# mratsim/constantine

Measured on NVIDIA H100. Metric: bls12_381_g1_msm_throughput, higher is better.
Workload: dtype u32

## Files before the change

constantine_b200/csrc/msm_affine.cuh:

```cuda
#pragma once
#include "ec.cuh"
#include "field_inv.cuh"

namespace b200 {

constexpr int AFF_MAX_LEVELS = 8;
constexpr uint32_t AFF_NONE = 0xFFFFFFFFu;

static __global__ void k_bucket_bounds(const uint32_t* __restrict__ keys, size_t n, uint32_t no_key, uint32_t* head, uint32_t* tail) {
  size_t q = (size_t)blockIdx.x * blockDim.x + threadIdx.x;
  if (q >= n) return;
  const uint32_t key = keys[q];
  if (key >= no_key) return;
  if (q == 0 || keys[q - 1] != key) head[key] = (uint32_t)q;
  if (q + 1 == n || keys[q + 1] != key) tail[key] = (uint32_t)(q + 1);
}

constexpr int SCAN_THREADS = 256, SCAN_PER_THREAD = 4, SCAN_ITEMS = SCAN_THREADS * SCAN_PER_THREAD;

B200_DEV uint32_t block_exclusive_scan(uint32_t v, uint32_t& total, uint32_t* smem ) {
  const unsigned lane = threadIdx.x & 31u, warp = threadIdx.x >> 5;
  uint32_t inc = v;
#pragma unroll
  for (int d = 1; d < 32; d <<= 1) {
    uint32_t t = __shfl_up_sync(0xFFFFFFFFu, inc, d);
    if (lane >= (unsigned)d) inc += t;
  }
  __syncthreads();
  if (lane == 31u) smem[warp] = inc;
  __syncthreads();
  uint32_t base = 0, tot = 0;
#pragma unroll
  for (int w = 0; w < SCAN_THREADS / 32; w++) {
    const uint32_t s = smem[w];
    if ((unsigned)w < warp) base += s;
    tot += s;
  }
  total = tot;
  return base + inc - v;
}

B200_DEV uint32_t level_count(uint32_t n, int r) { return (n + (1u << r) - 1u) >> r; }

static __global__ void __launch_bounds__(SCAN_THREADS) k_level_blocksums(const uint32_t* __restrict__ head, const uint32_t* __restrict__ tail,
                                                                          uint32_t nb, int L, uint32_t nblk, uint32_t* blocksum ) {
  __shared__ uint32_t sm[SCAN_THREADS / 32 + 1];
  const uint32_t b0 = blockIdx.x * SCAN_ITEMS + threadIdx.x * SCAN_PER_THREAD;
  uint32_t cnt[SCAN_PER_THREAD];
#pragma unroll
  for (int k = 0; k < SCAN_PER_THREAD; k++) cnt[k] = (b0 + k < nb) ? tail[b0 + k] - head[b0 + k] : 0u;
  for (int r = 0; r <= L; r++) {
    uint32_t s = 0;
#pragma unroll
    for (int k = 0; k < SCAN_PER_THREAD; k++) s += level_count(cnt[k], r);
    uint32_t tot;
    block_exclusive_scan(s, tot, sm);
    if (threadIdx.x == 0) blocksum[(size_t)r * nblk + blockIdx.x] = tot;
  }
}

static __global__ void __launch_bounds__(SCAN_THREADS) k_level_scan(uint32_t* blocksum, uint32_t nblk, int L, uint32_t nb, uint32_t* off) {
  __shared__ uint32_t sm[SCAN_THREADS / 32 + 1];
  for (int r = 0; r <= L; r++) {
    uint32_t carry = 0;
    for (uint32_t base = 0; base < nblk; base += SCAN_THREADS) {
      const uint32_t i = base + threadIdx.x;
      const uint32_t v = (i < nblk) ? blocksum[(size_t)r * nblk + i] : 0u;
      uint32_t tot;
      const uint32_t ex = block_exclusive_scan(v, tot, sm);
      if (i < nblk) blocksum[(size_t)r * nblk + i] = carry + ex;
      carry += tot;
    }
    if (threadIdx.x == 0) off[(size_t)r * (nb + 1) + nb] = carry;
  }
}

static __global__ void __launch_bounds__(SCAN_THREADS) k_level_offsets(const uint32_t* __restrict__ head, const uint32_t* __restrict__ tail,
                                                                        uint32_t nb, int L, uint32_t nblk, const uint32_t* __restrict__ blocksum,
                                                                        uint32_t* off) {
  __shared__ uint32_t sm[SCAN_THREADS / 32 + 1];
  const uint32_t b0 = blockIdx.x * SCAN_ITEMS + threadIdx.x * SCAN_PER_THREAD;
  uint32_t cnt[SCAN_PER_THREAD];
#pragma unroll
  for (int k = 0; k < SCAN_PER_THREAD; k++) cnt[k] = (b0 + k < nb) ? tail[b0 + k] - head[b0 + k] : 0u;
  for (int r = 0; r <= L; r++) {
    uint32_t c[SCAN_PER_THREAD], s = 0;
#pragma unroll
    for (int k = 0; k < SCAN_PER_THREAD; k++) { c[k] = level_count(cnt[k], r); s += c[k]; }
    uint32_t tot;
    uint32_t ex = block_exclusive_scan(s, tot, sm) + blocksum[(size_t)r * nblk + blockIdx.x];
#pragma unroll
    for (int k = 0; k < SCAN_PER_THREAD; k++) {
      if (b0 + k < nb) off[(size_t)r * (nb + 1) + b0 + k] = ex;
      ex += c[k];
    }
  }
}

struct AffinePlan {
  uint2* plan0;
  uint32_t* plan[AFF_MAX_LEVELS];
  uint32_t* surv_keys;
  uint32_t* surv_vals;
};

static __global__ void k_affine_plan(const uint32_t* __restrict__ keys, const uint32_t* __restrict__ vals, size_t n, uint32_t no_key,
                                     const uint32_t* __restrict__ head, const uint32_t* __restrict__ tail,
                                     const uint32_t* __restrict__ off, uint32_t nb, int L, AffinePlan P) {
  size_t q = (size_t)blockIdx.x * blockDim.x + threadIdx.x;
  if (q >= n) return;
  const uint32_t b = keys[q];
  if (b >= no_key) return;
  const uint32_t h = head[b], i = (uint32_t)q - h, cnt = tail[b] - h;
  const size_t stride = (size_t)nb + 1;
  for (int r = 0; r < L; r++) {
    if (i & ((2u << r) - 1u)) break;
    const uint32_t p = off[(size_t)(r + 1) * stride + b] + (i >> (r + 1));
    const uint32_t s = i >> r;
    const bool has2 = s + 1u < level_count(cnt, r);
    if (r == 0) P.plan0[p] = make_uint2(vals[q], has2 ? vals[q + 1] : AFF_NONE);
    else P.plan[r][p] = (off[(size_t)r * stride + b] + s) | (has2 ? 0x80000000u : 0u);
  }
  if ((i & ((1u << L) - 1u)) == 0u) {
    const uint32_t ps = off[(size_t)L * stride + b] + (i >> L);
    P.surv_keys[ps] = b;
    P.surv_vals[ps] = ps;
  }
}

template <class T>
B200_DEV Aff<T> load_affine_rw(const uint32_t* base, size_t idx) {
  const uint32_t* p = base + idx * (2 * T::WORDS);
  Aff<T> a;
  load_words_rw(a.x, p);
  load_words_rw(a.y, p + T::WORDS);
  return a;
}
template <class T>
B200_DEV void store_affine(uint32_t* base, size_t idx, const Aff<T>& a) {
  uint32_t* p = base + idx * (2 * T::WORDS);
  store_words(p, a.x);
  store_words(p + T::WORDS, a.y);
}

template <class T>
B200_DEV void scratch_store(uint4* scratch, size_t threads, size_t tid, uint32_t j, const T& v) {
  constexpr int V = T::WORDS / 4;
#pragma unroll
  for (int k = 0; k < V; k++) {
    uint4 w;
    w.x = v.word(4 * k + 0); w.y = v.word(4 * k + 1); w.z = v.word(4 * k + 2); w.w = v.word(4 * k + 3);
    scratch[((size_t)j * V + k) * threads + tid] = w;
  }
}
template <class T>
B200_DEV T scratch_load(const uint4* scratch, size_t threads, size_t tid, uint32_t j) {
  constexpr int V = T::WORDS / 4;
  T v;
#pragma unroll
  for (int k = 0; k < V; k++) {
    const uint4 w = scratch[((size_t)j * V + k) * threads + tid];
    v.set_word(4 * k + 0, w.x); v.set_word(4 * k + 1, w.y); v.set_word(4 * k + 2, w.z); v.set_word(4 * k + 3, w.w);
  }
  return v;
}

constexpr int PART_TILE = 1024, PART_THREADS = 256, PART_MAX = 8;

B200_DEV uint32_t pair_chunk(const uint2 task, uint32_t n_points, uint32_t P) {
  uint32_t idx = task.x & 0x7FFFFFFFu;
  if (task.y != AFF_NONE) { const uint32_t j = task.y & 0x7FFFFFFFu; if (j > idx) idx = j; }
  uint32_t q = (uint32_t)(((unsigned long long)idx * P) / n_points);
  return q < P ? q : P - 1u;
}

static __global__ void __launch_bounds__(PART_THREADS) k_part_count(const uint2* __restrict__ plan0, const uint32_t* __restrict__ total_ptr,
                                                                    uint32_t n_points, uint32_t P, uint32_t nblk, uint32_t* counts) {
  __shared__ uint32_t sm[PART_MAX];
  if (threadIdx.x < PART_MAX) sm[threadIdx.x] = 0;
  __syncthreads();
  const uint32_t total = *total_ptr;
  const uint32_t base = blockIdx.x * PART_TILE;
  uint32_t local[PART_MAX];
#pragma unroll
  for (int q = 0; q < PART_MAX; q++) local[q] = 0;
  for (uint32_t i = threadIdx.x; i < PART_TILE; i += PART_THREADS) {
    const uint32_t p = base + i;
    if (p < total) {
      const uint32_t q = pair_chunk(plan0[p], n_points, P);
#pragma unroll
      for (int k = 0; k < PART_MAX; k++) local[k] += (q == (uint32_t)k) ? 1u : 0u;
    }
  }
#pragma unroll
  for (int q = 0; q < PART_MAX; q++) {
    uint32_t v = local[q];
    for (int d = 16; d >= 1; d >>= 1) v += __shfl_xor_sync(0xFFFFFFFFu, v, d);
    if ((threadIdx.x & 31u) == 0 && v) atomicAdd(&sm[q], v);
  }
  __syncthreads();
  if (threadIdx.x < P) counts[threadIdx.x * nblk + blockIdx.x] = sm[threadIdx.x];
}

static __global__ void __launch_bounds__(SCAN_THREADS) k_part_scan(uint32_t* counts, uint32_t P, uint32_t nblk, uint32_t* starts) {
  __shared__ uint32_t sm[SCAN_THREADS / 32 + 1];
  uint32_t carry = 0;
  const uint32_t len = P * nblk;
  for (uint32_t base = 0; base < len; base += SCAN_THREADS) {
    const uint32_t i = base + threadIdx.x;
    const uint32_t v = (i < len) ? counts[i] : 0u;
    uint32_t tot;
    const uint32_t ex = block_exclusive_scan(v, tot, sm);
    if (i < len) {
      counts[i] = carry + ex;
      if (i % nblk == 0) starts[i / nblk] = carry + ex;
    }
    carry += tot;
  }
  if (threadIdx.x == 0) starts[P] = carry;
}

static __global__ void __launch_bounds__(PART_THREADS) k_part_scatter(const uint2* __restrict__ plan0, const uint32_t* __restrict__ total_ptr,
                                                                      uint32_t n_points, uint32_t P, uint32_t nblk,
                                                                      const uint32_t* __restrict__ offsets, uint32_t* perm) {
  __shared__ uint32_t warp_cnt[PART_THREADS / 32][PART_MAX];
  __shared__ uint32_t run_base[PART_MAX];
  const uint32_t total = *total_ptr;
  const unsigned lane = threadIdx.x & 31u, warp = threadIdx.x >> 5;
  if (threadIdx.x < PART_MAX) run_base[threadIdx.x] = (threadIdx.x < P) ? offsets[threadIdx.x * nblk + blockIdx.x] : 0u;
  __syncthreads();
  for (uint32_t round = 0; round < PART_TILE / PART_THREADS; round++) {
    const uint32_t p = blockIdx.x * PART_TILE + round * PART_THREADS + threadIdx.x;
    const bool live = p < total;
    const uint32_t q = live ? pair_chunk(plan0[p], n_points, P) : 0xFFFFFFFFu;
    uint32_t my_rank = 0;
    for (uint32_t k = 0; k < P; k++) {
      const unsigned m = __ballot_sync(0xFFFFFFFFu, q == k);
      if (q == k) my_rank = __popc(m & ((1u << lane) - 1u));
      if (lane == 0) warp_cnt[warp][k] = __popc(m);
    }
    __syncthreads();
    if (live) {
      uint32_t before = 0;
      for (unsigned w = 0; w < warp; w++) before += warp_cnt[w][q];
      perm[run_base[q] + before + my_rank] = p;
    }
    __syncthreads();
    if (threadIdx.x < P) {
      uint32_t tot = 0;
      for (unsigned w = 0; w < PART_THREADS / 32; w++) tot += warp_cnt[w][threadIdx.x];
      run_base[threadIdx.x] += tot;
    }
    __syncthreads();
  }
}

enum PairKind { PAIR_COPY1 = 0, PAIR_COPY2 = 1, PAIR_INF = 2, PAIR_ADD = 3, PAIR_DBL = 4 };

struct PairTask {
  uint32_t a, b;
};
template <bool FIRST>
B200_DEV PairTask load_task(const void* plan, size_t p) {
  PairTask t;
  if constexpr (FIRST) {
    const uint2 v = reinterpret_cast<const uint2*>(plan)[p];
    t.a = v.x; t.b = v.y;
  } else {
    const uint32_t v = reinterpret_cast<const uint32_t*>(plan)[p];
    t.a = v & 0x7FFFFFFFu;
    t.b = (v >> 31) ? t.a + 1u : AFF_NONE;
  }
  return t;
}
template <class T, bool FIRST>
B200_DEV T load_x(const uint32_t* src, uint32_t ref) {
  T x;
  if constexpr (FIRST) load_words(x, src + (size_t)(ref & 0x7FFFFFFFu) * (2 * T::WORDS));
  else load_words_rw(x, src + (size_t)ref * (2 * T::WORDS));
  return x;
}
template <class T, bool FIRST>
B200_DEV void decode_y(T& y, uint32_t ref, bool& zero) {
  zero = y.is_zero();
  if constexpr (FIRST) y.cneg((ref >> 31) != 0);
}
template <class T, bool FIRST>
B200_DEV T load_y(const uint32_t* src, uint32_t ref, bool& zero) {
  T y;
  if constexpr (FIRST) load_words(y, src + (size_t)(ref & 0x7FFFFFFFu) * (2 * T::WORDS) + T::WORDS);
  else load_words_rw(y, src + (size_t)ref * (2 * T::WORDS) + T::WORDS);
  decode_y<T, FIRST>(y, ref, zero);
  return y;
}

template <class T>
B200_DEV int classify_pair(bool single, const T& x1, const T& y1, bool inf1, const T& x2, const T& y2, bool inf2, T& den) {
  if (single) return PAIR_COPY1;
  if (inf1) return PAIR_COPY2;
  if (inf2) return PAIR_COPY1;
  den = x2 - x1;
  if (!den.is_zero()) return PAIR_ADD;
  if (!(y1 == y2) || y1.is_zero()) return PAIR_INF;
  den = y1.dbl();
  return PAIR_DBL;
}

template <class T, bool FIRST>
B200_DEV void pair_factor(const uint32_t* src, uint32_t a, uint32_t b, const T& x1, const T& x2, T& run) {
  const bool single = b == AFF_NONE;
  T den = x2 - x1;
  bool contributes = !single;
  if (!single && (den.is_zero() || x1.is_zero() || x2.is_zero())) {
    bool z1, z2;
    const T y1 = load_y<T, FIRST>(src, a, z1), y2 = load_y<T, FIRST>(src, b, z2);
    const int kind = classify_pair(false, x1, y1, z1 && x1.is_zero(), x2, y2, z2 && x2.is_zero(), den);
    contributes = kind >= PAIR_ADD;
  }
  if (contributes) run = run.mul_u(den);
}

template <class T, class Prefix>
B200_DEV Aff<T> pair_result(const Aff<T>& P1, bool z1, const Aff<T>& P2, bool z2, bool single, uint32_t j, T& inv, Prefix prefix) {
  T den;
  const int kind = classify_pair(single, P1.x, P1.y, z1 && P1.x.is_zero(), P2.x, P2.y, z2 && P2.x.is_zero(), den);
  Aff<T> R;
  if (kind < PAIR_ADD) {
    if (kind == PAIR_COPY1) R = P1;
    else if (kind == PAIR_COPY2) R = P2;
    else { R.x = T::zero(); R.y = T::zero(); }
  } else {
    T inv_den = inv;
    if (j > 0) inv_den = inv.mul_u(prefix());
    inv = inv.mul_u(den);
    T num;
    if (kind == PAIR_ADD) num = P2.y - P1.y;
    else { const T xx = P1.x.sqr(); num = xx.dbl() + xx; }
    const T lam = num.mul_u(inv_den);
    R.x = lam.sqr_u() - P1.x - P2.x;
    R.y = lam.mul_u(P1.x - R.x) - P1.y;
  }
  return R;
}

#ifndef B200_AFF_THREADS
#define B200_AFF_THREADS 128
#endif
#ifndef B200_AFF_MIN_BLOCKS
#define B200_AFF_MIN_BLOCKS 4
#endif

B200_DEV void prefetch_l2(const void* p) { asm volatile("prefetch.global.L2 [%0];" ::"l"(p)); }
B200_DEV void prefetch_span(const void* p, int bytes) {
  prefetch_l2(p);
  prefetch_l2((const char*)p + bytes - 1);
}
template <class T, bool FIRST>
B200_DEV void prefetch_point(const uint32_t* src, uint32_t ref) {
  const uint32_t idx = FIRST ? (ref & 0x7FFFFFFFu) : ref;
  prefetch_span(src + (size_t)idx * (2 * T::WORDS), 2 * T::WORDS * 4);
}

__host__ __device__ __forceinline__ size_t pair_rows(size_t slots, size_t threads) { return (slots + threads - 1) / threads; }

struct PairSlots {
  const uint32_t* perm;
  uint32_t total, M;
  B200_DEV PairSlots(const uint32_t* total_ptr, const uint32_t* perm_, const uint32_t* range, size_t threads) {
    const uint32_t range_begin = range ? range[0] : 0u;
    total = range ? range[1] - range[0] : *total_ptr;
    perm = perm_;
    if (perm) perm += range_begin;
    M = (uint32_t)pair_rows(total, threads);
  }
  B200_DEV size_t first(size_t tid) const { return (tid & ~(size_t)31) * M + (tid & 31u); }
  B200_DEV uint32_t count(size_t tid) const {
    const size_t f = first(tid);
    if (f >= total) return 0u;
    const uint32_t c = (uint32_t)(((size_t)total - f + 31) / 32);
    return c < M ? c : M;
  }
  B200_DEV size_t slot(size_t tid, uint32_t j) const {
    const size_t t = first(tid) + 32u * (size_t)j;
    return perm ? (size_t)perm[t] : t;
  }
};

template <class T, bool FIRST>
__global__ void __launch_bounds__(B200_AFF_THREADS, (T::WORDS <= 12) ? B200_AFF_MIN_BLOCKS : 1)
k_affine_pairs(const void* __restrict__ plan, const uint32_t* __restrict__ total_ptr, const uint32_t* src, uint32_t* dst, uint4* scratch,
               const uint32_t* __restrict__ perm = nullptr, const uint32_t* __restrict__ range = nullptr) {
  const size_t threads = (size_t)gridDim.x * blockDim.x;
  const size_t tid = (size_t)blockIdx.x * blockDim.x + threadIdx.x;
  const PairSlots S(total_ptr, perm, range, threads);
  const unsigned lane = threadIdx.x & 31u;
  if (S.count(tid - lane) == 0) return;
  const uint32_t cnt = S.count(tid);
  T run = T::one();
  {
    PairTask t_next = cnt ? load_task<FIRST>(plan, S.slot(tid, 0)) : PairTask{0u, AFF_NONE};
    T x1n = T::zero(), x2n = T::zero();
    if (cnt) {
      x1n = load_x<T, FIRST>(src, t_next.a);
      if (t_next.b != AFF_NONE) x2n = load_x<T, FIRST>(src, t_next.b);
    }
#pragma unroll 1
    for (uint32_t j = 0; j < cnt; j++) {
      const PairTask t = t_next;
      const T x1 = x1n, x2 = x2n;
      if (j + 1 < cnt) {
        t_next = load_task<FIRST>(plan, S.slot(tid, j + 1));
        x1n = load_x<T, FIRST>(src, t_next.a);
        if (t_next.b != AFF_NONE) x2n = load_x<T, FIRST>(src, t_next.b);
      }
      pair_factor<T, FIRST>(src, t.a, t.b, x1, x2, run);
      scratch_store(scratch, threads, tid, j, run);
    }
  }
  T inv = fe_inverse(run);
  size_t p_prev = cnt ? S.slot(tid, cnt - 1) : 0;
  PairTask t_prev = cnt ? load_task<FIRST>(plan, p_prev) : PairTask{0u, AFF_NONE};
#pragma unroll 1
  for (uint32_t jj = cnt; jj > 0; jj--) {
    const uint32_t j = jj - 1;
    const size_t p = p_prev;
    const PairTask t = t_prev;
    if (j > 0) {
      p_prev = S.slot(tid, j - 1);
      t_prev = load_task<FIRST>(plan, p_prev);
      prefetch_point<T, FIRST>(src, t_prev.a);
      if (t_prev.b != AFF_NONE) prefetch_point<T, FIRST>(src, t_prev.b);
      if (j > 1) {
        constexpr int V = T::WORDS / 4;
#pragma unroll
        for (int k = 0; k < V; k++) prefetch_l2(scratch + ((size_t)(j - 2) * V + k) * threads + tid);
      }
    }
    const bool single = t.b == AFF_NONE;
    Aff<T> P1, P2;
    bool z1 = false, z2 = false;
    P1.x = load_x<T, FIRST>(src, t.a);
    P1.y = load_y<T, FIRST>(src, t.a, z1);
    if (!single) {
      P2.x = load_x<T, FIRST>(src, t.b);
      P2.y = load_y<T, FIRST>(src, t.b, z2);
    } else {
      P2.x = T::zero(); P2.y = T::zero();
    }
    store_affine(dst, p, pair_result(P1, z1, P2, z2, single, j, inv, [&] { return scratch_load<T>(scratch, threads, tid, j - 1); }));
  }
}

#ifndef B200_AFF_WS_CONSUMERS
#define B200_AFF_WS_CONSUMERS 8
#endif
#ifndef B200_AFF_WS_STAGES
#define B200_AFF_WS_STAGES 2
#endif
constexpr int AFF_WS_CONSUMERS = B200_AFF_WS_CONSUMERS;
constexpr int AFF_WS_THREADS = 32 * (AFF_WS_CONSUMERS + 1);

template <class T>
struct AffRing {
  static constexpr bool USED = T::WORDS <= 12;
  static constexpr int V = T::WORDS / 4;
  static constexpr int S2 = B200_AFF_WS_STAGES;
  static constexpr int ROWS = S2 * 5 * V;
  static constexpr int S1 = ROWS / (2 * V);
  static constexpr size_t BYTES = (size_t)AFF_WS_CONSUMERS * ROWS * 32 * 16;
};

B200_DEV uint32_t smem_addr(const void* p) { return (uint32_t)__cvta_generic_to_shared(p); }
B200_DEV void mbar_init(uint64_t* b, uint32_t count) { asm volatile("mbarrier.init.shared::cta.b64 [%0], %1;" ::"r"(smem_addr(b)), "r"(count) : "memory"); }
B200_DEV void mbar_arrive(uint64_t* b) { asm volatile("mbarrier.arrive.shared::cta.b64 _, [%0];" ::"r"(smem_addr(b)) : "memory"); }
B200_DEV void mbar_wait(uint64_t* b, uint32_t parity) {
  asm volatile(
      "{\n\t.reg .pred P1;\n"
      "WAIT:\n\t"
      "mbarrier.try_wait.parity.shared::cta.b64 P1, [%0], %1;\n\t"
      "@!P1 bra WAIT;\n\t}" ::"r"(smem_addr(b)),
      "r"(parity)
      : "memory");
}
B200_DEV void cp_async_arrive(uint64_t* b) { asm volatile("cp.async.mbarrier.arrive.noinc.shared::cta.b64 [%0];" ::"r"(smem_addr(b)) : "memory"); }
B200_DEV void cp_async16(void* s, const void* g) { asm volatile("cp.async.cg.shared.global [%0], [%1], 16;" ::"r"(smem_addr(s)), "l"(g) : "memory"); }

template <class T>
B200_DEV void ring_fetch(uint4* ring, int row, unsigned lane, const uint32_t* g) {
#pragma unroll
  for (int k = 0; k < T::WORDS / 4; k++) cp_async16(ring + (row + k) * 32 + lane, g + 4 * k);
}
template <class T>
B200_DEV T ring_load(const uint4* ring, int row, unsigned lane) {
  T v;
#pragma unroll
  for (int k = 0; k < T::WORDS / 4; k++) {
    const uint4 w = ring[(row + k) * 32 + lane];
    v.set_word(4 * k + 0, w.x); v.set_word(4 * k + 1, w.y); v.set_word(4 * k + 2, w.z); v.set_word(4 * k + 3, w.w);
  }
  return v;
}

template <class T, bool FIRST>
__global__ void __launch_bounds__(AFF_WS_THREADS, 1)
k_affine_pairs_ws(const void* __restrict__ plan, const uint32_t* __restrict__ total_ptr, const uint32_t* src, uint32_t* dst, uint4* scratch,
                  const uint32_t* __restrict__ perm = nullptr, const uint32_t* __restrict__ range = nullptr) {
  using RG = AffRing<T>;
  constexpr int V = RG::V, NC = AFF_WS_CONSUMERS, S1 = RG::S1, S2 = RG::S2;
  extern __shared__ __align__(16) unsigned char aff_ring_raw[];
  __shared__ uint64_t full1[NC][S1], empty1[NC][S1], full2[NC][S2], empty2[NC][S2], drained[NC];
  __shared__ uint32_t s_task[NC][S1][3][32];
  const unsigned lane = threadIdx.x & 31u, warp = threadIdx.x >> 5;
  if (threadIdx.x == 0) {
    for (int w = 0; w < NC; w++) {
      for (int s = 0; s < S1; s++) { mbar_init(&full1[w][s], 64); mbar_init(&empty1[w][s], 32); }
      for (int s = 0; s < S2; s++) { mbar_init(&full2[w][s], 64); mbar_init(&empty2[w][s], 32); }
      mbar_init(&drained[w], 32);
    }
  }
  __syncthreads();
  const size_t threads = (size_t)gridDim.x * NC * 32;
  const PairSlots S(total_ptr, perm, range, threads);
  uint4* const ring_base = reinterpret_cast<uint4*>(aff_ring_raw);

  if (warp == NC) {
    uint32_t n[NC], cnt[NC];
#pragma unroll
    for (int w = 0; w < NC; w++) {
      const size_t tid = ((size_t)blockIdx.x * NC + w) * 32 + lane;
      n[w] = S.count(tid - lane);
      cnt[w] = S.count(tid);
    }
    auto tid_of = [&](int w) { return ((size_t)blockIdx.x * NC + w) * 32 + lane; };
    auto src_of = [&](uint32_t ref) { return src + (size_t)(FIRST ? (ref & 0x7FFFFFFFu) : ref) * (2 * T::WORDS); };
    uint32_t ta[NC], tb[NC], tp[NC];
    auto fetch_task = [&](int w, uint32_t j) {
      const size_t p = S.slot(tid_of(w), j);
      const PairTask t = load_task<FIRST>(plan, p);
      ta[w] = t.a; tb[w] = t.b; tp[w] = (uint32_t)p;
    };
#pragma unroll
    for (int w = 0; w < NC; w++) if (cnt[w]) fetch_task(w, 0);
#pragma unroll 1
    for (uint32_t j = 0; j < n[0]; j++) {
      uint32_t ca[NC], cb[NC];
#pragma unroll
      for (int w = 0; w < NC; w++) { ca[w] = ta[w]; cb[w] = tb[w]; }
#pragma unroll
      for (int w = 0; w < NC; w++) if (j + 1 < cnt[w]) fetch_task(w, j + 1);
#pragma unroll
      for (int w = 0; w < NC; w++) {
        if (j >= n[w]) continue;
        const int s = (int)(j % S1);
        mbar_wait(&empty1[w][s], ((j / S1) & 1u) ^ 1u);
        uint4* ring = ring_base + (size_t)w * RG::ROWS * 32;
        if (j < cnt[w]) {
          s_task[w][s][0][lane] = ca[w];
          s_task[w][s][1][lane] = cb[w];
          ring_fetch<T>(ring, s * 2 * V, lane, src_of(ca[w]));
          if (cb[w] != AFF_NONE) ring_fetch<T>(ring, s * 2 * V + V, lane, src_of(cb[w]));
        }
        cp_async_arrive(&full1[w][s]);
        mbar_arrive(&full1[w][s]);
      }
    }
#pragma unroll
    for (int w = 0; w < NC; w++) if (n[w] && n[w] - 1 < cnt[w]) fetch_task(w, n[w] - 1);
#pragma unroll 1
    for (uint32_t jj = 0; jj < n[0]; jj++) {
      uint32_t ca[NC], cb[NC], cp[NC];
#pragma unroll
      for (int w = 0; w < NC; w++) { ca[w] = ta[w]; cb[w] = tb[w]; cp[w] = tp[w]; }
#pragma unroll
      for (int w = 0; w < NC; w++) if (jj + 1 < n[w] && n[w] - 2 - jj < cnt[w]) fetch_task(w, n[w] - 2 - jj);
#pragma unroll
      for (int w = 0; w < NC; w++) {
        if (jj >= n[w]) continue;
        if (jj == 0) mbar_wait(&drained[w], 0);
        const uint32_t j = n[w] - 1 - jj;
        const int s = (int)(jj % S2);
        mbar_wait(&empty2[w][s], ((jj / S2) & 1u) ^ 1u);
        uint4* ring = ring_base + (size_t)w * RG::ROWS * 32;
        if (j < cnt[w]) {
          s_task[w][s][0][lane] = ca[w];
          s_task[w][s][1][lane] = cb[w];
          s_task[w][s][2][lane] = cp[w];
          const int row = s * 5 * V;
          ring_fetch<T>(ring, row, lane, src_of(ca[w]));
          ring_fetch<T>(ring, row + V, lane, src_of(ca[w]) + T::WORDS);
          if (cb[w] != AFF_NONE) {
            ring_fetch<T>(ring, row + 2 * V, lane, src_of(cb[w]));
            ring_fetch<T>(ring, row + 3 * V, lane, src_of(cb[w]) + T::WORDS);
          }
          if (j > 0) {
#pragma unroll
            for (int k = 0; k < V; k++)
              cp_async16(ring + (row + 4 * V + k) * 32 + lane, scratch + ((size_t)(j - 1) * V + k) * threads + tid_of(w));
          }
        }
        cp_async_arrive(&full2[w][s]);
        mbar_arrive(&full2[w][s]);
      }
    }
    asm volatile("cp.async.wait_all;" ::: "memory");
    return;
  }

  const size_t tid = ((size_t)blockIdx.x * NC + warp) * 32 + lane;
  const uint32_t n = S.count(tid - lane), cnt = S.count(tid);
  if (n == 0) return;
  const uint4* ring = ring_base + (size_t)warp * RG::ROWS * 32;
  T run = T::one();
#pragma unroll 1
  for (uint32_t j = 0; j < n; j++) {
    const int s = (int)(j % S1);
    mbar_wait(&full1[warp][s], (j / S1) & 1u);
    const uint32_t a = s_task[warp][s][0][lane], b = s_task[warp][s][1][lane];
    const T x1 = ring_load<T>(ring, s * 2 * V, lane), x2 = ring_load<T>(ring, s * 2 * V + V, lane);
    mbar_arrive(&empty1[warp][s]);
    if (j >= cnt) continue;
    pair_factor<T, FIRST>(src, a, b, x1, x2, run);
    scratch_store(scratch, threads, tid, j, run);
  }
  mbar_arrive(&drained[warp]);
  T inv = fe_inverse(run);
#pragma unroll 1
  for (uint32_t jj = 0; jj < n; jj++) {
    const uint32_t j = n - 1 - jj;
    const int s = (int)(jj % S2);
    mbar_wait(&full2[warp][s], (jj / S2) & 1u);
    const int row = s * 5 * V;
    const uint32_t a = s_task[warp][s][0][lane], b = s_task[warp][s][1][lane], p = s_task[warp][s][2][lane];
    const bool single = b == AFF_NONE;
    Aff<T> P1, P2;
    P1.x = ring_load<T>(ring, row, lane);
    P1.y = ring_load<T>(ring, row + V, lane);
    P2.x = single ? T::zero() : ring_load<T>(ring, row + 2 * V, lane);
    P2.y = single ? T::zero() : ring_load<T>(ring, row + 3 * V, lane);
    const T pre = ring_load<T>(ring, row + 4 * V, lane);
    mbar_arrive(&empty2[warp][s]);
    if (j >= cnt) continue;
    bool z1, z2 = false;
    decode_y<T, FIRST>(P1.y, a, z1);
    if (!single) decode_y<T, FIRST>(P2.y, b, z2);
    store_affine(dst, p, pair_result(P1, z1, P2, z2, single, j, inv, [&] { return pre; }));
  }
}

template <class T>
struct PairKernel {
  static constexpr bool WS = AffRing<T>::USED;
  static constexpr int THREADS = WS ? AFF_WS_THREADS : B200_AFF_THREADS;
  static constexpr int SLOT_THREADS = WS ? 32 * AFF_WS_CONSUMERS : B200_AFF_THREADS;
  static constexpr int SMEM = WS ? (int)AffRing<T>::BYTES : 0;
  template <bool FIRST>
  static auto entry() {
    if constexpr (WS) return k_affine_pairs_ws<T, FIRST>;
    else return k_affine_pairs<T, FIRST>;
  }
};

template <class T>
cudaError_t affine_pairs_blocks_per_sm(int* bps) {
  using K = PairKernel<T>;
  int b[2] = {0, 0};
  cudaError_t e;
  for (int f = 0; f < 2; f++) {
    const auto k = f == 0 ? K::template entry<true>() : K::template entry<false>();
    if (K::SMEM && (e = cudaFuncSetAttribute(k, cudaFuncAttributeMaxDynamicSharedMemorySize, K::SMEM)) != cudaSuccess) return e;
    if ((e = cudaOccupancyMaxActiveBlocksPerMultiprocessor(&b[f], k, K::THREADS, K::SMEM)) != cudaSuccess) return e;
  }
  *bps = b[1] < b[0] ? b[1] : b[0];
  return cudaSuccess;
}

template <class T, bool FIRST>
void launch_affine_pairs(unsigned grid, cudaStream_t s, const void* plan, const uint32_t* total_ptr, const uint32_t* src, uint32_t* dst, uint4* scratch,
                         const uint32_t* perm = nullptr, const uint32_t* range = nullptr) {
  using K = PairKernel<T>;
  K::template entry<FIRST>()<<<grid, K::THREADS, K::SMEM, s>>>(plan, total_ptr, src, dst, scratch, perm, range);
}

}
```

Before: 114.7.

## Split affine pair producer work across multiple producer warps

Replaces the single producer warp that fed all consumer warps with a configurable number of producer warps, defaulting to two. Each producer handles an equal group of consumers, issuing the task loads and cp.async fetches only for its group. This is meant to stop the lone producer from becoming the bottleneck that serialises loads for eight consumers. The cost is one extra warp per block, which adds register and scheduling pressure under launch bounds of one block per SM.

Result: faster. 117.5 (median of 6 runs) (+2.4%).

```diff
diff --git a/constantine_b200/csrc/msm_affine.cuh b/constantine_b200/csrc/msm_affine.cuh
--- a/constantine_b200/csrc/msm_affine.cuh
+++ b/constantine_b200/csrc/msm_affine.cuh
@@ -457,8 +457,13 @@
 #ifndef B200_AFF_WS_STAGES
 #define B200_AFF_WS_STAGES 2
 #endif
+#ifndef B200_AFF_WS_PRODUCERS
+#define B200_AFF_WS_PRODUCERS 2
+#endif
 constexpr int AFF_WS_CONSUMERS = B200_AFF_WS_CONSUMERS;
-constexpr int AFF_WS_THREADS = 32 * (AFF_WS_CONSUMERS + 1);
+constexpr int AFF_WS_PRODUCERS = B200_AFF_WS_PRODUCERS;
+static_assert(AFF_WS_CONSUMERS % AFF_WS_PRODUCERS == 0, "each producer warp serves the same number of consumer warps");
+constexpr int AFF_WS_THREADS = 32 * (AFF_WS_CONSUMERS + AFF_WS_PRODUCERS);
 
 template <class T>
 struct AffRing {
@@ -506,7 +511,7 @@
 k_affine_pairs_ws(const void* __restrict__ plan, const uint32_t* __restrict__ total_ptr, const uint32_t* src, uint32_t* dst, uint4* scratch,
                   const uint32_t* __restrict__ perm = nullptr, const uint32_t* __restrict__ range = nullptr) {
   using RG = AffRing<T>;
-  constexpr int V = RG::V, NC = AFF_WS_CONSUMERS, S1 = RG::S1, S2 = RG::S2;
+  constexpr int V = RG::V, NC = AFF_WS_CONSUMERS, NG = NC / AFF_WS_PRODUCERS, S1 = RG::S1, S2 = RG::S2;
   extern __shared__ __align__(16) unsigned char aff_ring_raw[];
   __shared__ uint64_t full1[NC][S1], empty1[NC][S1], full2[NC][S2], empty2[NC][S2], drained[NC];
   __shared__ uint32_t s_task[NC][S1][3][32];
@@ -523,79 +528,81 @@
   const PairSlots S(total_ptr, perm, range, threads);
   uint4* const ring_base = reinterpret_cast<uint4*>(aff_ring_raw);
 
-  if (warp == NC) {
-    uint32_t n[NC], cnt[NC];
-#pragma unroll
-    for (int w = 0; w < NC; w++) {
-      const size_t tid = ((size_t)blockIdx.x * NC + w) * 32 + lane;
-      n[w] = S.count(tid - lane);
-      cnt[w] = S.count(tid);
-    }
-    auto tid_of = [&](int w) { return ((size_t)blockIdx.x * NC + w) * 32 + lane; };
+  if (warp >= NC) {
+    const int w0 = (int)(warp - NC) * NG;
+    auto tid_of = [&](int i) { return ((size_t)blockIdx.x * NC + w0 + i) * 32 + lane; };
+    uint32_t n[NG], cnt[NG];
+#pragma unroll
+    for (int i = 0; i < NG; i++) {
+      n[i] = S.count(tid_of(i) - lane);
+      cnt[i] = S.count(tid_of(i));
+    }
     auto src_of = [&](uint32_t ref) { return src + (size_t)(FIRST ? (ref & 0x7FFFFFFFu) : ref) * (2 * T::WORDS); };
-    uint32_t ta[NC], tb[NC], tp[NC];
-    auto fetch_task = [&](int w, uint32_t j) {
-      const size_t p = S.slot(tid_of(w), j);
+    uint32_t ta[NG], tb[NG], tp[NG];
+    auto fetch_task = [&](int i, uint32_t j) {
+      const size_t p = S.slot(tid_of(i), j);
       const PairTask t = load_task<FIRST>(plan, p);
-      ta[w] = t.a; tb[w] = t.b; tp[w] = (uint32_t)p;
+      ta[i] = t.a; tb[i] = t.b; tp[i] = (uint32_t)p;
     };
 #pragma unroll
-    for (int w = 0; w < NC; w++) if (cnt[w]) fetch_task(w, 0);
+    for (int i = 0; i < NG; i++) if (cnt[i]) fetch_task(i, 0);
 #pragma unroll 1
     for (uint32_t j = 0; j < n[0]; j++) {
-      uint32_t ca[NC], cb[NC];
-#pragma unroll
-      for (int w = 0; w < NC; w++) { ca[w] = ta[w]; cb[w] = tb[w]; }
-#pragma unroll
-      for (int w = 0; w < NC; w++) if (j + 1 < cnt[w]) fetch_task(w, j + 1);
-#pragma unroll
-      for (int w = 0; w < NC; w++) {
-        if (j >= n[w]) continue;
+      uint32_t ca[NG], cb[NG];
+#pragma unroll
+      for (int i = 0; i < NG; i++) { ca[i] = ta[i]; cb[i] = tb[i]; }
+#pragma unroll
+      for (int i = 0; i < NG; i++) if (j + 1 < cnt[i]) fetch_task(i, j + 1);
+#pragma unroll
+      for (int i = 0; i < NG; i++) {
+        if (j >= n[i]) continue;
+        const int w = w0 + i;
         const int s = (int)(j % S1);
         mbar_wait(&empty1[w][s], ((j / S1) & 1u) ^ 1u);
         uint4* ring = ring_base + (size_t)w * RG::ROWS * 32;
-        if (j < cnt[w]) {
-          s_task[w][s][0][lane] = ca[w];
-          s_task[w][s][1][lane] = cb[w];
-          ring_fetch<T>(ring, s * 2 * V, lane, src_of(ca[w]));
-          if (cb[w] != AFF_NONE) ring_fetch<T>(ring, s * 2 * V + V, lane, src_of(cb[w]));
+        if (j < cnt[i]) {
+          s_task[w][s][0][lane] = ca[i];
+          s_task[w][s][1][lane] = cb[i];
+          ring_fetch<T>(ring, s * 2 * V, lane, src_of(ca[i]));
+          if (cb[i] != AFF_NONE) ring_fetch<T>(ring, s * 2 * V + V, lane, src_of(cb[i]));
         }
         cp_async_arrive(&full1[w][s]);
         mbar_arrive(&full1[w][s]);
       }
     }
 #pragma unroll
-    for (int w = 0; w < NC; w++) if (n[w] && n[w] - 1 < cnt[w]) fetch_task(w, n[w] - 1);
+    for (int i = 0; i < NG; i++) if (n[i] && n[i] - 1 < cnt[i]) fetch_task(i, n[i] - 1);
 #pragma unroll 1
     for (uint32_t jj = 0; jj < n[0]; jj++) {
-      uint32_t ca[NC], cb[NC], cp[NC];
-#pragma unroll
-      for (int w = 0; w < NC; w++) { ca[w] = ta[w]; cb[w] = tb[w]; cp[w] = tp[w]; }
-#pragma unroll
-      for (int w = 0; w < NC; w++) if (jj + 1 < n[w] && n[w] - 2 - jj < cnt[w]) fetch_task(w, n[w] - 2 - jj);
-#pragma unroll
-      for (int w = 0; w < NC; w++) {
-        if (jj >= n[w]) continue;
+      uint32_t ca[NG], cb[NG], cp[NG];
+#pragma unroll
+      for (int i = 0; i < NG; i++) { ca[i] = ta[i]; cb[i] = tb[i]; cp[i] = tp[i]; }
+#pragma unroll
+      for (int i = 0; i < NG; i++) if (jj + 1 < n[i] && n[i] - 2 - jj < cnt[i]) fetch_task(i, n[i] - 2 - jj);
+#pragma unroll
+      for (int i = 0; i < NG; i++) {
+        if (jj >= n[i]) continue;
+        const int w = w0 + i;
         if (jj == 0) mbar_wait(&drained[w], 0);
-        const uint32_t j = n[w] - 1 - jj;
+        const uint32_t j = n[i] - 1 - jj;
         const int s = (int)(jj % S2);
         mbar_wait(&empty2[w][s], ((jj / S2) & 1u) ^ 1u);
         uint4* ring = ring_base + (size_t)w * RG::ROWS * 32;
-        if (j < cnt[w]) {
-          s_task[w][s][0][lane] = ca[w];
-          s_task[w][s][1][lane] = cb[w];
-          s_task[w][s][2][lane] = cp[w];
+        if (j < cnt[i]) {
+          s_task[w][s][0][lane] = ca[i];
+          s_task[w][s][1][lane] = cb[i];
+          s_task[w][s][2][lane] = cp[i];
           const int row = s * 5 * V;
-          ring_fetch<T>(ring, row, lane, src_of(ca[w]));
-          ring_fetch<T>(ring, row + V, lane, src_of(ca[w]) + T::WORDS);
-          if (cb[w] != AFF_NONE) {
-            ring_fetch<T>(ring, row + 2 * V, lane, src_of(cb[w]));
-            ring_fetch<T>(ring, row + 3 * V, lane, src_of(cb[w]) + T::WORDS);
+          ring_fetch<T>(ring, row, lane, src_of(ca[i]));
+          ring_fetch<T>(ring, row + V, lane, src_of(ca[i]) + T::WORDS);
+          if (cb[i] != AFF_NONE) {
+            ring_fetch<T>(ring, row + 2 * V, lane, src_of(cb[i]));
+            ring_fetch<T>(ring, row + 3 * V, lane, src_of(cb[i]) + T::WORDS);
           }
           if (j > 0) {
 #pragma unroll
             for (int k = 0; k < V; k++)
-              cp_async16(ring + (row + 4 * V + k) * 32 + lane, scratch + ((size_t)(j - 1) * V + k) * threads + tid_of(w));
+              cp_async16(ring + (row + 4 * V + k) * 32 + lane, scratch + ((size_t)(j - 1) * V + k) * threads + tid_of(i));
           }
         }
         cp_async_arrive(&full2[w][s]);
```
